# kalenforn/clip-based-cross-modal-hash

Measured on AMD Instinct MI355X. Metric: Hamming query x gallery pairs/sec (fused mAP@all pass, DCMHT COCO-shaped 64-bit), higher is better.
Workload: dtype u32; 1 GPU; configs[1] DCMHT COCO 64-bit retrieval: Q=5000 queries x R=117218 gallery items per GPU (x1 GPUs, contiguous shards), K=64 bits, C=80 classes, mAP@all; Q=5000, R_per_gpu=117218, K=64, C=80, parallelism=gallery-shard x1, query_blocks=1

## Files before the change

### clip-based-cross-modal-hash_amd/csrc/xmh_scan.hip

```cpp
#include "xmh_common.h"
#include <atomic>
#include <math.h>
#include <mutex>
#include <string.h>
#include <vector>
#include "xmh_scan_bits.h"
#include "xmh_scan_mfma.h"
#include "xmh_scan_kernels.h"

#include <stdlib.h>
#include <type_traits>

namespace {

constexpr int kSlotBudget64 = 9 * 1024;
constexpr int kSlotBudget32 = 5 * 1024;
constexpr int slots_for(int W, bool tern, int counter_bytes) {
    const int nbmax = (tern ? 64 : 32) * W + 1;
    const int budget = counter_bytes == 8 ? kSlotBudget64 : kSlotBudget32;
    const int cap = W > 8 ? 64 : 8;
    int S = 2;
    while (S < cap && nbmax * (64 / S) * counter_bytes > budget) S *= 2;
    return S;
}
// ... 350 lines not shown
        break;
    }
    case Kern::kApC: snprintf(out, n, "k_scan_ap_c<false, %d, %s>", l.eb, tf[l.half]); break;
    case Kern::kApR2: snprintf(out, n, "k_scan_ap_r2<%d, %d, %d, false>", l.nml, l.NW, l.S); break;
    }
    return XMH_OK;
}

int check_common(const char* who, const ScanCall& c, const xmh_scan_plan& p) {
    if (!c.qbits || !c.rbits || !c.qlab || !c.rlab || !c.ws) return xmh::fail(XMH_EINVAL, "%s: null pointer", who);
    if ((c.qzero == nullptr) != (c.rzero == nullptr)) return xmh::fail(XMH_EINVAL, "%s: zero masks must be given for both sides or neither", who);
    if (c.C <= 0) return xmh::fail(XMH_EINVAL, "%s: C=%d", who, c.C);
    const size_t need = ws_layout(p, 0).total;
    if (c.ws_bytes < need) return xmh::fail(XMH_EINVAL, "%s: workspace too small (%zu < %zu; %zu with the pair cache)", who, c.ws_bytes, need, (size_t)p.ws_bytes);
    return XMH_OK;
}

ScanArgs make_args(const ScanCall& c, const xmh_scan_plan& p) {
    return ScanArgs{c.qbits, c.qzero, c.qlab, c.rbits, c.rzero, c.rlab, (int)c.Q, (int)c.R, c.K, (int)p.chunk, (int)p.nchunk, (int)p.nqtile, (int)p.qpad,
                    (int)p.nbuckets, nullptr, (int)p.nqtile};
}

MfmaArgs r2_args(const ScanCall& c, const Launch& l, const xmh_scan_plan& p, int nqt) {
    MfmaArgs a{c.qbits, (int)c.Q, (int)c.R, c.K, l.W, (int)p.chunk, (int)p.nchunk, nqt, (int)p.nbuckets, (int)p.qpad};
    a.rbits = c.rbits; a.rlab = c.rlab; a.qlab = c.qlab; a.LW = l.LW;
    return a;
}

struct Geom { unsigned grid, block; size_t lds; int nqt, nrun; };
Geom launch_geom(const Launch& l, const xmh_scan_plan& p, int64_t Q) {
    const size_t nb = (size_t)p.nbuckets;
    const bool ap = l.kern == Kern::kApS || l.kern == Kern::kApC || l.kern == Kern::kApR2;
    Geom g{0, 64u * (unsigned)l.NW, 0, 0};
    if (l.kern == Kern::kHistS || l.kern == Kern::kApS) {
        g.lds = ((nb * (64 / l.S) * (ap && !l.p32 ? 2 : 1) + 3) & ~(size_t)3) * 4 * l.NW + (ap && l.cache ? 0 : aos_ring_bytes(l.W, l.LW, l.tern));
        g.nqt = (int)p.nqtile * l.S / l.NW;
    } else if (l.kern == Kern::kApC) {
        g.lds = nb * (64 / l.S) * 8; g.nqt = (int)p.nqtile * l.S;
    } else if (l.kern == Kern::kHistB) {
        g.nqt = (int)(p.qpad / (16 * kMfmaWaves));
    } else {
        g.lds = (size_t)l.NW * l.S * nb * 16 * (ap ? 8 : 4); g.nqt = (int)(p.qpad / (l.NW * l.S * 16));
    }
    g.nrun = g.nqt;
    if (ap) {
        static const bool all_tiles = xmh_experiment_env("XMH_AP_TILES") && atoi(xmh_experiment_env("XMH_AP_TILES")) == 0;
        if (!all_tiles) g.nrun = (int)xmh::ceil_div(Q, p.qpad / g.nqt);
    }
    g.grid = xmh::scan_grid_blocks(g.nrun, (int)p.nchunk);
    return g;
}

template <typename KernT, typename... Args>
int start(const char* who, const Launch& l, const Geom& g, hipStream_t st, KernT kern, int S, int NW, bool cache, Args... args) {
    if (l.S != S || l.NW != NW || l.cache != cache)
        return xmh::fail(XMH_ENOTSUP, "%s: the route names an instance with S=%d NW=%d cache=%d, the one compiled for W=%d LW=%d has S=%d NW=%d cache=%d", who, l.S,
                         l.NW, (int)l.cache, l.W, l.LW, S, NW, (int)cache);
    if (const int rc = xmh::raise_dynamic_lds(reinterpret_cast<const void*>(kern), g.lds, who)) return rc;
    hipLaunchKernelGGL(kern, dim3(g.grid), dim3(g.block), g.lds, st, args...);
    return XMH_OK;
}

struct ScanCtx {
    const ScanCall& c;
    hipStream_t st;
    xmh_scan_plan p;
    ScanRoute r;
    WsLayout L;
    ScanArgs a;
    uint32_t kcap = 0xffffffffu;
    bool capped = false;
    template <typename T> T* at(size_t off) const { return reinterpret_cast<T*>(static_cast<char*>(c.ws) + off); }
    uint32_t* chunk_hist() const { return at<uint32_t>(L.chunk_hist); }
    const uint2* below() const { return at<uint2>(L.below); }
    uint2* tot() const { return at<uint2>(L.tot); }
    uint2* dpre() const { return at<uint2>(L.dpre); }
    uint32_t* cap_ws() const { return at<uint32_t>(L.cap); }
    float* ap_part() const { return at<float>(L.ap_part); }
    ScanArgs args(const Geom& g, bool cached) const { ScanArgs as = a; as.nqt = g.nqt; as.nrun = g.nrun; as.pair_cache = cached ? pair_cache() : nullptr; return as; }
    uint32_t* gate(int word = 0) const { return at<uint32_t>(L.gate) + word; }
    const uint32_t* gate_if(const Launch& l, unsigned g, int word) const { return (l.gate & g) ? gate(word) : nullptr; }
    uint4* pair_cache() const { return r.cache_bytes ? at<uint4>(L.pair_cache) : nullptr; }
};

int plan_call(const char* who, ScanCtx& x, const Overrides& ov) {
    if (const int rc = make_plan(x.c.Q, x.c.R, x.c.K, x.c.tern, &x.p, ov)) return rc;
    return check_common(who, x.c, x.p);
}
void route_call(ScanCtx& x, Mode mode, const Overrides& ov) {
    x.r = scan_route(x.p, x.c, mode, ov, x.st);
    x.a = make_args(x.c, x.p);
    x.L = ws_layout(x.p, x.r.cache_bytes);
}

int valu_hist(const ScanCtx& x) {
    const Launch& h = x.r.p1;
    const Geom g = launch_geom(h, x.p, x.c.Q);
    const ScanArgs as = x.args(g, h.cache);
    auto go = [&](auto kern, int S, int NW, bool cache) {
        xmh::ProfScope prof("scan_hist", x.st);
        return start("xmh_hamming_hist", h, g, x.st, kern, S, NW, cache, as, x.chunk_hist());
    };
    auto launch = [&](auto tern_c) {
        constexpr bool T = decltype(tern_c)::value;
        return dispatch_shape<T>(h.W, h.LW, [&](auto w, auto l) {
            constexpr int WW = decltype(w)::value, LL = decltype(l)::value;
            if constexpr (kPairCacheShape<WW, T>) {
                if (h.cache) return go(k_scan_hist_s<WW, LL, T, cache_slots(WW), 1, true>, cache_slots(WW), 1, true);
            }
            constexpr int S = slots_for(WW, T, 4);
            constexpr int NW = S == 64 ? waves_for(WW, T) : 1;
            return go(k_scan_hist_s<WW, LL, T, S, NW, false>, S, NW, false);
        });
    };
    return h.tern ? launch(std::true_type{}) : launch(std::false_type{});
}

int mfma_hist(const ScanCtx& x) {
    const Launch& h = x.r.p1;
    const xmh_scan_plan& p = x.p;
    const Geom g = launch_geom(h, p, x.c.Q);
    uint32_t* chunk_hist = x.chunk_hist();
    uint4* cache = x.pair_cache();
    if (h.kern == Kern::kHistB) {
        xmh::ScanBitsArgs a{x.c.rbits, x.c.rlab, x.c.qbits, x.c.qlab, (int)x.c.Q, (int)x.c.R, x.c.K, h.W, h.LW, (int)p.chunk, (int)p.nchunk, g.nqt,
                            (int)p.nbuckets, (int)p.qpad};
        a.rzero = x.c.rzero; a.qzero = x.c.qzero;
        return xmh::launch_scan_hist_bits(a, h.S, chunk_hist, cache, x.st);
    }
    hipLaunchKernelGGL(k_scan_touch, dim3(xmh::scan_grid_blocks(kTouchPerChunk, (int)p.nchunk)), dim3(256), 0, x.st, x.c.rbits, x.c.rlab, x.c.R, h.W, h.LW,
                       p.chunk, (int)p.nchunk, x.at<uint32_t>(x.L.tick), (int)((x.L.gate + 256 - x.L.tick) / 4));
    XMH_LAUNCH_CHECK("xmh_hamming_hist control words");
    const MfmaArgs a = r2_args(x.c, h, p, g.nqt);
    xmh::ProfScope prof("scan_hist", x.st);
    auto go = [&](auto kern, int NW, int NQ, bool cached, auto... wrap_word) { return start("xmh_hamming_hist", h, g, x.st, kern, NQ, NW, cached, a, chunk_hist, cache, wrap_word...); };
    if (h.kern == Kern::kHistR2w) {
        uint32_t* ovf = x.gate(kGateWrapped);
        return h.nml == 1 ? (h.cache ? go(k_scan_hist_r2w<1, 4, 2, true>, 4, 2, true, ovf) : go(k_scan_hist_r2w<1, 4, 2, false>, 4, 2, false, ovf))
                          : (h.cache ? go(k_scan_hist_r2w<2, 4, 2, true>, 4, 2, true, ovf) : go(k_scan_hist_r2w<2, 4, 2, false>, 4, 2, false, ovf));
    }
    return h.nml == 1 ? (h.cache ? go(k_scan_hist_r2<1, 4, 4, true>, 4, 4, true) : go(k_scan_hist_r2<1, 4, 4, false>, 4, 4, false))
                      : (h.cache ? go(k_scan_hist_r2<2, 4, 4, true>, 4, 4, true) : go(k_scan_hist_r2<2, 4, 4, false>, 4, 4, false));
}

int hamming_hist_impl(const ScanCall& c, uint32_t* hist_all, uint32_t* hist_rel, xmh_stream_t stream, const Overrides& ov) {
    ScanCtx x{c, xmh::as_stream(stream)};
    if (const int rc = plan_call("xmh_hamming_hist", x, ov)) return rc;
    route_call(x, Mode::kUnsharded, ov);
    const xmh_scan_plan& p = x.p;
    const Kern kern = x.r.p1.kern;
    if (kern == Kern::kHistS || kern == Kern::kHistB) XMH_HIP(hipMemsetAsync(x.at<char>(x.L.tick), 0, x.L.gate + 256 - x.L.tick, x.st));
    if (const int rc = kern == Kern::kHistS ? valu_hist(x) : mfma_hist(x)) return rc;
    XMH_LAUNCH_CHECK("xmh_hamming_hist");
    hipLaunchKernelGGL(k_scan_below, dim3((unsigned)p.nqtile, (unsigned)xmh::ceil_div(p.nbuckets, 4)), dim3(256), 0, x.st, x.chunk_hist(), (int)p.qpad,
                       (int)p.nbuckets, (int)p.nchunk, kern != Kern::kHistS ? kRelHi16 : 0u, x.at<uint2>(x.L.below), x.tot(), x.at<uint32_t>(x.L.tick), (int)c.Q, x.dpre(),
                       x.cap_ws(), x.gate(), hist_all, hist_rel);
    XMH_LAUNCH_CHECK("xmh_hamming_hist below");
    return XMH_OK;
}

}

extern "C" int xmh_scan_plan_make(int64_t Q, int64_t R, int K, int ternary, xmh_scan_plan* plan_host) {
    if (!plan_host) return xmh::fail(XMH_EINVAL, "xmh_scan_plan_make: null plan");
    return make_plan(Q, R, K, ternary, plan_host);
}

extern "C" size_t xmh_scan_pair_cache_bytes(int64_t Q, int64_t R, int K, int ternary) {
    xmh_scan_plan p;
    if (make_plan(Q, R, K, ternary, &p)) return 0;
    return pair_cache_bytes(p, K, ternary != 0, pass1_family(K, ternary != 0, {}));
}

extern "C" size_t xmh_scan_pair_cache_offset(int64_t Q, int64_t R, int K, int ternary) {
    xmh_scan_plan p;
    if (make_plan(Q, R, K, ternary, &p)) return (size_t)-1;
    return ws_layout(p, 0).pair_cache;
}

extern "C" size_t xmh_scan_ws_bytes_nocache(int64_t Q, int64_t R, int K, int ternary) {
    xmh_scan_plan p;
    if (make_plan(Q, R, K, ternary, &p)) return 0;
    return ws_layout(p, 0).total;
}

extern "C" int xmh_scan_describe(int64_t Q, int64_t R, int K, int C, int ternary, char* out, size_t out_bytes) {
    if (!out || out_bytes < 64) return xmh::fail(XMH_EINVAL, "xmh_scan_describe: buffer too small");
    xmh_scan_plan p;
    if (const int rc = make_plan(Q, R, K, ternary, &p)) return rc;
    Overrides ov;
    ov.describe = true;
    const ScanCall c{nullptr, nullptr, nullptr, nullptr, nullptr, nullptr, Q, R, K, C, nullptr, (size_t)p.ws_bytes, ternary != 0};
    const ScanRoute r = scan_route(p, c, Mode::kUnsharded, ov, nullptr);
    char p1[160], p2[200] = "", one[120];
    if (const int rc = describe_launch(r.p1, p1, sizeof(p1))) return rc;
    for (const bool p32 : {true, false})
        for (int i = 0; i < r.n2; ++i) {
            if (r.p2[i].stand_in || r.p2[i].p32 != p32) continue;
            if (const int rc = describe_launch(r.p2[i], one, sizeof(one))) return rc;
            const size_t at = strlen(p2);
            snprintf(p2 + at, sizeof(p2) - at, "%s%s", at ? "|" : "", one);
        }
    if ((size_t)snprintf(out, out_bytes, "pass1=%s;pass2=%s", p1, p2) >= out_bytes) return xmh::fail(XMH_EINVAL, "xmh_scan_describe: buffer too small");
    return XMH_OK;
}

extern "C" int xmh_hamming_hist(const uint32_t* qbits, const uint32_t* qzero, const uint32_t* qlab,
                                const uint32_t* rbits, const uint32_t* rzero, const uint32_t* rlab, int64_t Q, int64_t R,
                                int K, int C, void* ws, size_t ws_bytes, uint32_t* hist_all, uint32_t* hist_rel,
                                xmh_stream_t stream) {
    XMH_RANGE("xmh_hamming_hist (pass 1)");
    const ScanCall c{qbits, qzero, qlab, rbits, rzero, rlab, Q, R, K, C, ws, ws_bytes, qzero != nullptr};
    return hamming_hist_impl(c, hist_all, hist_rel, stream, {});
}

namespace {
int ap_offsets(const ScanCtx& x, const Pass2& o) {
    const xmh_scan_plan& p = x.p;
    if (o.mode == Mode::kUnsharded) return XMH_OK;
    if (o.mode == Mode::kAllToAll)
        hipLaunchKernelGGL(k_shard_scatter_offsets, dim3((unsigned)xmh::ceil_div(p.qpad, 256), (unsigned)p.nbuckets + 1), dim3(256), 0, x.st,
                           reinterpret_cast<const uint2*>(o.hist_g), (int)p.nbuckets, (int)(p.qpad / o.world), (int)x.c.Q, (int)p.qpad, o.k, x.dpre(), x.cap_ws(),
                           o.cap, x.gate(2));
    else if (o.mode == Mode::kTotals)
        hipLaunchKernelGGL(k_shard_offsets_dpre, dim3((unsigned)p.nqtile), dim3(256), 0, x.st, reinterpret_cast<const uint2*>(o.hist_g), o.world, o.rank,
                           (int)x.c.Q, (int)p.qpad, (int)p.nbuckets, o.k, x.dpre(), x.cap_ws(), o.cap, x.gate(2));
    else
        hipLaunchKernelGGL(k_scan_dpre, dim3((unsigned)p.nqtile), dim3(256), 0, x.st, (const uint2*)x.tot(), (int)x.c.Q, (int)p.qpad, (int)p.nbuckets, o.base_all,
                           o.base_rel, o.nrel_total, o.k, x.dpre(), x.cap_ws(), o.cap, (uint32_t*)nullptr, (uint32_t*)nullptr, (uint32_t*)nullptr, x.gate(2));
    XMH_LAUNCH_CHECK(o.mode == Mode::kAllToAll ? "xmh_hamming_map_sharded_offsets scatter" : (o.mode == Mode::kTotals ? "xmh_hamming_map_sharded offsets" : "xmh_hamming_ap dpre"));
    return XMH_OK;
}

int ap_launch_c(const ScanCtx& x, const Launch& l) {
    const Geom g = launch_geom(l, x.p, x.c.Q);
    const ScanArgs as = x.args(g, true);
    xmh::ProfScope prof("scan_ap", x.st);
    auto go = [&](auto kc, int S) {
        return start("xmh_hamming_ap", l, g, x.st, kc, S, 1, l.cache, as, x.below(), (const uint2*)x.dpre(), (const uint32_t*)x.cap_ws(), x.ap_part(),
                     x.gate_if(l, kBySize, 2), x.kcap, x.gate_if(l, kByWrap, kGateWrapped), x.gate_if(l, kByWidth, 0), l.gate & kByWidth ? x.r.rank_bits : 0);
    };
    if (l.eb == 16) return x.capped ? go(k_scan_ap_c<true, 16>, 8) : go(k_scan_ap_c<false, 16>, 8);
    if (l.half) return x.capped ? go(k_scan_ap_c<true, 8, true>, 8) : go(k_scan_ap_c<false, 8, true>, 8);
    return x.capped ? go(k_scan_ap_c<true, 8>, 4) : go(k_scan_ap_c<false, 8>, 4);
}

int ap_launch_r2(const ScanCtx& x, const Launch& l) {
    const Geom g = launch_geom(l, x.p, x.c.Q);
    const MfmaArgs ma = r2_args(x.c, l, x.p, g.nrun);
    xmh::ProfScope prof("scan_ap", x.st);
    auto go = [&](auto kern) {
        return start("xmh_hamming_ap", l, g, x.st, kern, kAp2Groups, kAp2Waves, l.cache, ma, x.below(), (const uint2*)x.dpre(), (const uint32_t*)x.cap_ws(), x.ap_part(),
                     x.gate_if(l, kBySize, 2), x.kcap);
    };
    return l.nml == 1 ? (x.capped ? go(k_scan_ap_r2<1, kAp2Waves, kAp2Groups, true>) : go(k_scan_ap_r2<1, kAp2Waves, kAp2Groups, false>))
                      : (x.capped ? go(k_scan_ap_r2<2, kAp2Waves, kAp2Groups, true>) : go(k_scan_ap_r2<2, kAp2Waves, kAp2Groups, false>));
}

int ap_launch_s(const ScanCtx& x, const Launch& l) {
    const Geom g = launch_geom(l, x.p, x.c.Q);
    const ScanArgs as = x.args(g, l.cache);
    auto go = [&](auto kern, int S, int NW, bool cache, const uint32_t* run_if) {
        xmh::ProfScope prof(l.p32 ? "scan_ap32" : "scan_ap", x.st);
        return start("xmh_hamming_ap", l, g, x.st, kern, S, NW, cache, as, x.below(), (const uint2*)x.dpre(), (const uint32_t*)x.cap_ws(), x.ap_part(),
                     (const uint32_t*)x.gate(), x.r.rank_bits, x.kcap, x.gate_if(l, kBySize, 2), run_if);
    };
    auto by_shape = [&](auto tern_c, auto cap_c, auto p32_c, auto masked_c) {
        constexpr bool T = decltype(tern_c)::value, CP = decltype(cap_c)::value, P32 = decltype(p32_c)::value, MK = decltype(masked_c)::value;
        return dispatch_shape<T>(l.W, l.LW, [&](auto w, auto lw) {
            constexpr int WW = decltype(w)::value, LL = decltype(lw)::value;
            if constexpr (P32 && MK) return xmh::fail(XMH_ENOTSUP, "xmh_hamming_ap: the masked fallback runs 64-bit counters only");
            else {
                if constexpr (kPairCacheShape<WW, T> && !MK) {
                    if (l.cache)
                        return go(k_scan_ap_s<WW, 1, T, CP, cache_slots(WW), P32, MK, 1, true>, cache_slots(WW), 1, true, nullptr);
                }
                (void)CP;
                constexpr int S = slots_for(WW, T, P32 ? 4 : 8);
                constexpr int NW = S == 64 ? waves_for(WW, T) : 1;
                return go(k_scan_ap_s<WW, LL, T, true, S, P32, MK, NW, false>, S, NW, false, x.gate_if(l, kByWrap, kGateWrapped));
            }
        });
    };
    using T1 = std::true_type; using T0 = std::false_type;
    auto by_mask = [&](auto t, auto c, auto w) { return l.masked ? by_shape(t, c, w, T1{}) : by_shape(t, c, w, T0{}); };
    auto by_width = [&](auto t, auto c) { return l.p32 ? by_mask(t, c, T1{}) : by_mask(t, c, T0{}); };
    auto by_cap = [&](auto t) { return x.capped ? by_width(t, T1{}) : by_width(t, T0{}); };
    return l.tern ? by_cap(T1{}) : by_cap(T0{});
}

int ap_reduce(const ScanCtx& x, const Pass2& o) {
    const int64_t Q = x.c.Q;
    const unsigned nred = (unsigned)xmh::ceil_div(Q, 64);
    if (o.map_out && nred <= 4096) {
        hipLaunchKernelGGL(k_ap_reduce_map, dim3(nred), dim3(256), 0, x.st, (const float*)x.ap_part(), (int)Q, (int)x.p.qpad, (int)x.p.nchunk,
                           (const uint32_t*)x.cap_ws(), x.kcap, o.cap, o.ap_sum, x.at<double>(x.L.gate + 256), x.gate(1), o.map_out);
        XMH_LAUNCH_CHECK("xmh_hamming_map reduce+finalize");
        return XMH_OK;
    }
    hipLaunchKernelGGL(k_ap_reduce, dim3(nred), dim3(256), 0, x.st, (const float*)x.ap_part(), (int)Q, (int)x.p.qpad, (int)x.p.nchunk, o.ap_sum,
                       o.mode != Mode::kUnsharded ? (const uint32_t*)nullptr : (const uint32_t*)x.cap_ws(), x.kcap, o.cap);
    XMH_LAUNCH_CHECK("xmh_hamming_ap reduce");
    if (o.map_out) {
        hipLaunchKernelGGL(k_map_finalize, dim3(1), dim3(256), 0, x.st, (const double*)o.ap_sum, (const int32_t*)o.cap, Q, o.map_out);
        XMH_LAUNCH_CHECK("xmh_hamming_map finalize");
    }
    return XMH_OK;
// ... 243 lines not shown
```

### clip-based-cross-modal-hash_amd/csrc/xmh_scan_kernels.h

```cpp
#pragma once
#include "xmh_scan_mfma.h"

namespace {
template <int W, int LW, bool TERN>
struct QueryRegs {
    uint32_t b[W];
    uint32_t z[TERN ? W : 1];
    uint32_t l[LW];
    __device__ __forceinline__ void load(const ScanArgs& a, int q) {
        const bool ok = q < a.Q;
#pragma unroll
        for (int w = 0; w < W; ++w) b[w] = ok ? a.qbits[(int64_t)q * W + w] : 0u;
        if (TERN) {
#pragma unroll
            for (int w = 0; w < W; ++w) z[w] = ok ? a.qzero[(int64_t)q * W + w] : 0xffffffffu;
        }
#pragma unroll
        for (int w = 0; w < LW; ++w) l[w] = ok ? a.qlab[(int64_t)q * LW + w] : 0u;
    }
};

template <int W, int LW, bool TERN>
struct Rec {
    uint32_t b[W];
    uint32_t z[TERN ? W : 1];
    uint32_t l[LW];
};

template <int W, int LW, bool TERN>
__device__ __forceinline__ void rec_eval01(const QueryRegs<W, LW, TERN>& qr, const Rec<W, LW, TERN>& r, int K, int& d, uint32_t& hit01) {
    if (!TERN) {
        int acc = 0;
#pragma unroll
        for (int w = 0; w < W; ++w) acc += __popc(qr.b[w] ^ r.b[w]);
        d = acc;
    } else {
        int live_n = 0, diff_n = 0;
#pragma unroll
        for (int w = 0; w < W; ++w) {
            const uint32_t live = ~(qr.z[w] | r.z[w]);
            live_n += __popc(live);
            diff_n += __popc((qr.b[w] ^ r.b[w]) & live);
        }
        d = K - live_n + 2 * diff_n;
    }
    uint32_t hit = qr.l[0] & r.l[0];
#pragma unroll
    for (int w = 1; w < LW; ++w) asm("v_and_or_b32 %0, %1, %2, %0" : "+v"(hit) : "v"(qr.l[w]), "v"(r.l[w]));
    asm("v_min_u32 %0, %1, 1" : "=v"(hit01) : "v"(hit));
}

constexpr uint32_t kRelHi16 = 0xffffffffu;
constexpr int kGateWrapped = 3;
__global__ __launch_bounds__(256) void k_scan_below(const uint32_t* __restrict__ chunk_hist, int qpad, int nb, int nchunk, uint32_t rel_scale,
                                                    uint2* __restrict__ below, uint2* __restrict__ tot, uint32_t* __restrict__ tickets, int Q,
                                                    uint2* __restrict__ dpre, uint32_t* __restrict__ nrel_ws, uint32_t* __restrict__ nrel_max,
                                                    uint32_t* __restrict__ hist_all, uint32_t* __restrict__ hist_rel) {
    __shared__ uint2 part[4][64];
    __shared__ int last;
    const int lane = threadIdx.x & 63, wq = threadIdx.x >> 6;
    const int d = blockIdx.y * 4 + wq;
    const int q = blockIdx.x * 64 + lane;
    const bool hi16 = rel_scale == kRelHi16;
    if (d < nb) {
        uint32_t ra = 0, rr = 0;
        int c = 0;
        for (; c + 4 <= nchunk; c += 4) {
            uint32_t h[4];
#pragma unroll
            for (int j = 0; j < 4; ++j) h[j] = chunk_hist[((int64_t)(c + j) * nb + d) * qpad + q];
#pragma unroll
            for (int j = 0; j < 4; ++j) {
                below[((int64_t)(c + j) * nb + d) * qpad + q] = make_uint2(ra, rr);
                const uint32_t rel = hi16 ? h[j] & 0xffffu : (rel_scale ? h[j] / rel_scale : h[j] >> 16);
                ra += hi16 ? h[j] >> 16 : (rel_scale ? h[j] - rel * rel_scale : h[j] & 0xffffu);
                rr += rel;
            }
        }
        for (; c < nchunk; ++c) {
            const uint32_t h = chunk_hist[((int64_t)c * nb + d) * qpad + q];
            below[((int64_t)c * nb + d) * qpad + q] = make_uint2(ra, rr);
            const uint32_t rel = hi16 ? h & 0xffffu : (rel_scale ? h / rel_scale : h >> 16);
            ra += hi16 ? h >> 16 : (rel_scale ? h - rel * rel_scale : h & 0xffffu);
            rr += rel;
        }
        __hip_atomic_store(reinterpret_cast<unsigned long long*>(tot + (int64_t)d * qpad + q), (unsigned long long)ra | ((unsigned long long)rr << 32),
                           __ATOMIC_RELAXED, __HIP_MEMORY_SCOPE_AGENT);
    }
    if (!tickets) return;
    asm volatile("s_waitcnt vmcnt(0)" ::: "memory");
    __syncthreads();
    if (threadIdx.x == 0) {
        const uint32_t t = __hip_atomic_fetch_add(tickets + blockIdx.x, 1u, __ATOMIC_RELAXED, __HIP_MEMORY_SCOPE_AGENT);
        last = t == gridDim.y - 1;
    }
    __syncthreads();
    if (!last) return;
    auto tot_at = [&](int dd) {
        const unsigned long long v = __hip_atomic_load(reinterpret_cast<const unsigned long long*>(tot + (int64_t)dd * qpad + q), __ATOMIC_RELAXED,
                                                       __HIP_MEMORY_SCOPE_AGENT);
        return make_uint2((uint32_t)v, (uint32_t)(v >> 32));
    };
    const int nbq = (nb + 3) / 4;
    const int d0 = wq * nbq, d1 = (d0 + nbq < nb) ? d0 + nbq : nb;
    uint32_t sa = 0, sr = 0;
    for (int dd = d0; dd < d1; dd += 8) {
        uint2 t[8];
#pragma unroll
        for (int j = 0; j < 8; ++j) t[j] = dd + j < d1 ? tot_at(dd + j) : make_uint2(0u, 0u);
#pragma unroll
        for (int j = 0; j < 8; ++j) { sa += t[j].x; sr += t[j].y; }
    }
    part[wq][lane] = make_uint2(sa, sr);
    __syncthreads();
    uint32_t ra = 0, rr = 0, tr = 0;
#pragma unroll
    for (int w = 0; w < 4; ++w) {
        const uint2 pw = part[w][lane];
        if (w < wq) { ra += pw.x; rr += pw.y; }
        tr += pw.y;
    }
    for (int dd = d0; dd < d1; dd += 8) {
        uint2 t[8];
#pragma unroll
        for (int j = 0; j < 8; ++j) t[j] = dd + j < d1 ? tot_at(dd + j) : make_uint2(0u, 0u);
#pragma unroll
        for (int j = 0; j < 8; ++j) {
            if (dd + j < d1) {
                dpre[(int64_t)(dd + j) * qpad + q] = make_uint2(ra, rr);
                if (hist_all && q < Q) hist_all[(int64_t)q * nb + dd + j] = t[j].x;
                if (hist_rel && q < Q) hist_rel[(int64_t)q * nb + dd + j] = t[j].y;
                ra += t[j].x;
                rr += t[j].y;
            }
        }
    }
    if (wq == 0) {
        nrel_ws[q] = tr;
        if (q < Q) atomicMax(nrel_max, tr);
    }
}

__global__ __launch_bounds__(256) void k_scan_dpre(const uint2* __restrict__ tot, int Q, int qpad, int nb,
                                                   const uint32_t* __restrict__ base_all,
                                                   const uint32_t* __restrict__ base_rel,
                                                   const uint32_t* __restrict__ nrel_total, int64_t kcap,
                                                   uint2* __restrict__ dpre, uint32_t* __restrict__ cap_ws,
                                                   int32_t* __restrict__ cap_out, uint32_t* __restrict__ hist_all,
                                                   uint32_t* __restrict__ hist_rel, uint32_t* __restrict__ nrel_max,
                                                   uint32_t* __restrict__ rank_max = nullptr) {
    __shared__ uint2 part[4][64];
    const int lane = threadIdx.x & 63, wq = threadIdx.x >> 6;
    const int q = blockIdx.x * 64 + lane;
    const bool qok = q < Q;
    const int nbq = (nb + 3) / 4;
    const int d0 = wq * nbq, d1 = (d0 + nbq < nb) ? d0 + nbq : nb;
    uint32_t sa = 0, sr = 0;
    for (int d = d0; d < d1; d += 8) {
        uint2 t[8];
#pragma unroll
        for (int j = 0; j < 8; ++j) t[j] = d + j < d1 ? tot[(int64_t)(d + j) * qpad + q] : make_uint2(0u, 0u);
#pragma unroll
        for (int j = 0; j < 8; ++j) { sa += t[j].x; sr += t[j].y; }
    }
    part[wq][lane] = make_uint2(sa, sr);
    __syncthreads();
    uint32_t ra = 0, rr = 0, ta = 0, tr = 0, rmax = 0;
#pragma unroll
    for (int w = 0; w < 4; ++w) {
        const uint2 p = part[w][lane];
        if (w < wq) { ra += p.x; rr += p.y; }
        ta += p.x; tr += p.y;
    }
    for (int d = d0; d < d1; d += 8) {
        uint2 t[8];
#pragma unroll
        for (int j = 0; j < 8; ++j) t[j] = d + j < d1 ? tot[(int64_t)(d + j) * qpad + q] : make_uint2(0u, 0u);
#pragma unroll
        for (int j = 0; j < 8; ++j) {
            if (d + j < d1) {
                uint2 o = make_uint2(ra, rr);
                if (base_all && qok) {
                    o = make_uint2(base_all[(int64_t)q * nb + d + j], base_rel[(int64_t)q * nb + d + j]);
                    rmax = max(rmax, o.x + t[j].x);
                }
                if (dpre) dpre[(int64_t)(d + j) * qpad + q] = o;
                if (qok && hist_all) hist_all[(int64_t)q * nb + d + j] = t[j].x;
                if (qok && hist_rel) hist_rel[(int64_t)q * nb + d + j] = t[j].y;
                ra += t[j].x;
                rr += t[j].y;
            }
        }
    }
    if (cap_ws && wq == 0) {
        const uint32_t nrel = nrel_total ? (qok ? nrel_total[q] : 0u) : tr;
        const uint32_t cap = (kcap > 0 && (uint64_t)kcap < (uint64_t)nrel) ? (uint32_t)kcap : nrel;
        cap_ws[q] = nrel;
        if (qok && cap_out) cap_out[q] = (int32_t)cap;
        if (qok && nrel_max) atomicMax(nrel_max, nrel);
    }
    if (rank_max) {
        for (int o = 32; o; o >>= 1) rmax = max(rmax, (uint32_t)__shfl_xor((int)rmax, o));
        if (lane == 0 && rmax) atomicMax(rank_max, rmax);
    }
    (void)ta;
}

template <int W, int LW, bool TERN>
struct AosBatch {
    static constexpr int RW = W * (TERN ? 2 : 1) + LW;
    static constexpr int RS = (RW + 3) / 4 * 4;
    using R = Rec<W, LW, TERN>;
    static constexpr bool COAL = W >= 16 && !TERN;
    uint32_t w[RS];
    template <int NW = 1>
    __device__ __forceinline__ void load(const ScanArgs& a, int64_t base, int64_t hi, int lane, int wave = 0) {
        const int64_t i = base + lane;
        const bool ok = i < hi;
        if (COAL) {
#pragma unroll
            for (int jj = 0; jj < W / 4 / NW; ++jj) {
                const int o = (jj * NW + wave) * 256 + lane * 4;
                const bool okj = base + o / W < hi;
                const uint4 v = okj ? *reinterpret_cast<const uint4*>(a.rbits + base * W + o) : make_uint4(0u, 0u, 0u, 0u);
                w[4 * jj] = v.x; w[4 * jj + 1] = v.y; w[4 * jj + 2] = v.z; w[4 * jj + 3] = v.w;
            }
        } else {
#pragma unroll
            for (int x = 0; x < W; ++x) w[x] = ok ? a.rbits[i * W + x] : 0u;
        }
        if (TERN) {
#pragma unroll
            for (int x = 0; x < W; ++x) w[W + x] = ok ? a.rzero[i * W + x] : 0xffffffffu;
        }
        if (NW == 1 || wave == 0) {
#pragma unroll
            for (int x = 0; x < LW; ++x) w[W * (TERN ? 2 : 1) + x] = ok ? a.rlab[i * LW + x] : 0u;
        }
#pragma unroll
        for (int x = RW; x < RS; ++x) w[x] = 0u;
    }
    template <int NW = 1>
    __device__ __forceinline__ void publish(uint32_t* ring, int lane, int wave = 0) const {
        if (COAL) {
#pragma unroll
            for (int jj = 0; jj < W / 4 / NW; ++jj) {
                const int o = (jj * NW + wave) * 256 + lane * 4;
                *reinterpret_cast<uint4*>(ring + (o / W) * RS + (o % W)) = make_uint4(w[4 * jj], w[4 * jj + 1], w[4 * jj + 2], w[4 * jj + 3]);
            }
            if (NW == 1 || wave == 0)
                *reinterpret_cast<uint4*>(ring + lane * RS + W) = make_uint4(w[W], w[W + 1], w[W + 2], w[W + 3]);
            return;
        }
#pragma unroll
        for (int x = 0; x < RS; x += 4) *reinterpret_cast<uint4*>(ring + lane * RS + x) = make_uint4(w[x], w[x + 1], w[x + 2], w[x + 3]);
    }
    static __device__ __forceinline__ void get(R& r, const uint32_t* mine, int off_dwords) {
        uint32_t t[RS];
#pragma unroll
        for (int x = 0; x < RS; x += 4) {
            if (x + 4 <= RW || RW - x > 2) {
                const uint4 v = *reinterpret_cast<const uint4*>(mine + off_dwords + x);
                t[x] = v.x; t[x + 1] = v.y; t[x + 2] = v.z; t[x + 3] = v.w;
            } else if (RW - x == 2) {
                const uint2 v = *reinterpret_cast<const uint2*>(mine + off_dwords + x);
                t[x] = v.x; t[x + 1] = v.y; t[x + 2] = 0u; t[x + 3] = 0u;
            } else {
                t[x] = mine[off_dwords + x]; t[x + 1] = 0u; t[x + 2] = 0u; t[x + 3] = 0u;
            }
        }
#pragma unroll
        for (int x = 0; x < W; ++x) r.b[x] = t[x];
        if (TERN) {
#pragma unroll
            for (int x = 0; x < W; ++x) r.z[x] = t[W + x];
        }
#pragma unroll
        for (int x = 0; x < LW; ++x) r.l[x] = t[W * (TERN ? 2 : 1) + x];
    }
};

template <int S> struct SlotGeom {
    static constexpr int QW = 64 / S;
    static constexpr int LOG_QW = QW == 64 ? 6 : (QW == 32 ? 5 : (QW == 16 ? 4 : (QW == 8 ? 3 : (QW == 4 ? 2 : (QW == 2 ? 1 : 0)))));
    static constexpr int G = QW >= 16 ? 8 : (QW < 4 ? QW : 4);
    static constexpr int NG = QW / G;
};
// ... 670 lines not shown
```

Before: 1738 billion pairs/s.

## Widen k_scan_below to two queries per lane and batch chunk loads

Each lane in k_scan_below now handles two adjacent queries using uint2 loads and uint4 stores. Each wave covers two buckets, so the grid's y dimension halves. Chunk-histogram loads are issued in batches of 32 before a single vmcnt wait, and field extraction uses bitfield-extract instead of the divide/mask path. The last-block prefix pass loads all bucket totals once into registers when they fit, instead of reading tot twice. The intent is to raise memory-level parallelism and cut instruction and load overhead in this scan. In exchange it assumes the 16/16 packed format: the old general rel_scale divide path is replaced by shifts, and register pressure rises.

```diff
diff --git a/clip-based-cross-modal-hash_amd/csrc/xmh_scan.hip b/clip-based-cross-modal-hash_amd/csrc/xmh_scan.hip
--- a/clip-based-cross-modal-hash_amd/csrc/xmh_scan.hip
+++ b/clip-based-cross-modal-hash_amd/csrc/xmh_scan.hip
@@ -526,7 +526,7 @@
     if (kern == Kern::kHistS || kern == Kern::kHistB) XMH_HIP(hipMemsetAsync(x.at<char>(x.L.tick), 0, x.L.gate + 256 - x.L.tick, x.st));
     if (const int rc = kern == Kern::kHistS ? valu_hist(x) : mfma_hist(x)) return rc;
     XMH_LAUNCH_CHECK("xmh_hamming_hist");
-    hipLaunchKernelGGL(k_scan_below, dim3((unsigned)p.nqtile, (unsigned)xmh::ceil_div(p.nbuckets, 4)), dim3(256), 0, x.st, x.chunk_hist(), (int)p.qpad,
+    hipLaunchKernelGGL(k_scan_below, dim3((unsigned)p.nqtile, (unsigned)xmh::ceil_div(p.nbuckets, 8)), dim3(256), 0, x.st, x.chunk_hist(), (int)p.qpad,
                        (int)p.nbuckets, (int)p.nchunk, kern != Kern::kHistS ? kRelHi16 : 0u, x.at<uint2>(x.L.below), x.tot(), x.at<uint32_t>(x.L.tick), (int)c.Q, x.dpre(),
                        x.cap_ws(), x.gate(), hist_all, hist_rel);
     XMH_LAUNCH_CHECK("xmh_hamming_hist below");
diff --git a/clip-based-cross-modal-hash_amd/csrc/xmh_scan_kernels.h b/clip-based-cross-modal-hash_amd/csrc/xmh_scan_kernels.h
--- a/clip-based-cross-modal-hash_amd/csrc/xmh_scan_kernels.h
+++ b/clip-based-cross-modal-hash_amd/csrc/xmh_scan_kernels.h
@@ -51,6 +51,9 @@
 }
 
 constexpr uint32_t kRelHi16 = 0xffffffffu;
+constexpr int kBelowRound = 32;
+constexpr int kTotRound = 36;
+constexpr int kWaitVm0 = 0x0F70;
 constexpr int kGateWrapped = 3;
 __global__ __launch_bounds__(256) void k_scan_below(const uint32_t* __restrict__ chunk_hist, int qpad, int nb, int nchunk, uint32_t rel_scale,
                                                     uint2* __restrict__ below, uint2* __restrict__ tot, uint32_t* __restrict__ tickets, int Q,
@@ -58,34 +61,51 @@
                                                     uint32_t* __restrict__ hist_all, uint32_t* __restrict__ hist_rel) {
     __shared__ uint2 part[4][64];
     __shared__ int last;
-    const int lane = threadIdx.x & 63, wq = threadIdx.x >> 6;
-    const int d = blockIdx.y * 4 + wq;
-    const int q = blockIdx.x * 64 + lane;
-    const bool hi16 = rel_scale == kRelHi16;
-    if (d < nb) {
-        uint32_t ra = 0, rr = 0;
-        int c = 0;
-        for (; c + 4 <= nchunk; c += 4) {
-            uint32_t h[4];
-#pragma unroll
-            for (int j = 0; j < 4; ++j) h[j] = chunk_hist[((int64_t)(c + j) * nb + d) * qpad + q];
-#pragma unroll
-            for (int j = 0; j < 4; ++j) {
-                below[((int64_t)(c + j) * nb + d) * qpad + q] = make_uint2(ra, rr);
-                const uint32_t rel = hi16 ? h[j] & 0xffffu : (rel_scale ? h[j] / rel_scale : h[j] >> 16);
-                ra += hi16 ? h[j] >> 16 : (rel_scale ? h[j] - rel * rel_scale : h[j] & 0xffffu);
-                rr += rel;
-            }
-        }
-        for (; c < nchunk; ++c) {
-            const uint32_t h = chunk_hist[((int64_t)c * nb + d) * qpad + q];
-            below[((int64_t)c * nb + d) * qpad + q] = make_uint2(ra, rr);
-            const uint32_t rel = hi16 ? h & 0xffffu : (rel_scale ? h / rel_scale : h >> 16);
-            ra += hi16 ? h >> 16 : (rel_scale ? h - rel * rel_scale : h & 0xffffu);
-            rr += rel;
-        }
-        __hip_atomic_store(reinterpret_cast<unsigned long long*>(tot + (int64_t)d * qpad + q), (unsigned long long)ra | ((unsigned long long)rr << 32),
-                           __ATOMIC_RELAXED, __HIP_MEMORY_SCOPE_AGENT);
+    const int lane = threadIdx.x & 63, wq = __builtin_amdgcn_readfirstlane(threadIdx.x >> 6);
+    const uint32_t sh_all = rel_scale == kRelHi16 ? 16u : 0u, sh_rel = 16u - sh_all;
+    {
+        const int d = blockIdx.y * 8 + wq * 2 + (lane >> 5);
+        const int q2 = blockIdx.x * 64 + (lane & 31) * 2;
+        if (d < nb) {
+            const int64_t cs = (int64_t)nb * qpad;
+            const int64_t corner = (int64_t)blockIdx.y * 8 * qpad + blockIdx.x * 64;
+            const uint32_t off = (uint32_t)((wq * 2 + (lane >> 5)) * qpad + (lane & 31) * 2) * 4u;
+            const char* __restrict__ src = reinterpret_cast<const char*>(chunk_hist + corner);
+            char* __restrict__ dst = reinterpret_cast<char*>(below + corner);
+            int64_t step = cs * 4;
+            uint32_t a0 = 0, r0 = 0, a1 = 0, r1 = 0;
+            auto round = [&](int left) {
+                uint2 h[kBelowRound];
+#pragma unroll
+                for (int g = 0; g < kBelowRound; g += 8) {
+                    if (g < left) {
+#pragma unroll
+                        for (int j = g; j < g + 8; ++j) h[j] = *reinterpret_cast<const uint2*>(src + (j < left ? j : left - 1) * step + off);
+                    }
+                }
+                __builtin_amdgcn_s_waitcnt(kWaitVm0);
+#pragma unroll
+                for (int j = 0; j < kBelowRound; ++j) {
+                    if (j < left) {
+                        *reinterpret_cast<uint4*>(dst + 2 * j * step + 2u * off) = make_uint4(a0, r0, a1, r1);
+                        a0 += __builtin_amdgcn_ubfe(h[j].x, sh_all, 16);
+                        r0 += __builtin_amdgcn_ubfe(h[j].x, sh_rel, 16);
+                        a1 += __builtin_amdgcn_ubfe(h[j].y, sh_all, 16);
+                        r1 += __builtin_amdgcn_ubfe(h[j].y, sh_rel, 16);
+                    }
+                }
+                src += kBelowRound * step;
+                dst += 2 * kBelowRound * step;
+            };
+            round(nchunk);
+            for (int c0 = kBelowRound; c0 < nchunk; c0 += kBelowRound) {
+                asm volatile("" : "+s"(step));
+                round(nchunk - c0);
+            }
+            unsigned long long* t2 = reinterpret_cast<unsigned long long*>(tot + (int64_t)d * qpad + q2);
+            __hip_atomic_store(t2, (unsigned long long)a0 | ((unsigned long long)r0 << 32), __ATOMIC_RELAXED, __HIP_MEMORY_SCOPE_AGENT);
+            __hip_atomic_store(t2 + 1, (unsigned long long)a1 | ((unsigned long long)r1 << 32), __ATOMIC_RELAXED, __HIP_MEMORY_SCOPE_AGENT);
+        }
     }
     if (!tickets) return;
     asm volatile("s_waitcnt vmcnt(0)" ::: "memory");
@@ -96,43 +116,81 @@
     }
     __syncthreads();
     if (!last) return;
+    const int q = blockIdx.x * 64 + lane;
+    const uint32_t qoff = (uint32_t)lane * 8u;
+    const int64_t rowb = (int64_t)qpad * 8;
     auto tot_at = [&](int dd) {
-        const unsigned long long v = __hip_atomic_load(reinterpret_cast<const unsigned long long*>(tot + (int64_t)dd * qpad + q), __ATOMIC_RELAXED,
-                                                       __HIP_MEMORY_SCOPE_AGENT);
+        const char* row = reinterpret_cast<const char*>(tot + blockIdx.x * 64) + dd * rowb;
+        const unsigned long long v = __hip_atomic_load(reinterpret_cast<const unsigned long long*>(row + qoff), __ATOMIC_RELAXED, __HIP_MEMORY_SCOPE_AGENT);
         return make_uint2((uint32_t)v, (uint32_t)(v >> 32));
     };
     const int nbq = (nb + 3) / 4;
     const int d0 = wq * nbq, d1 = (d0 + nbq < nb) ? d0 + nbq : nb;
-    uint32_t sa = 0, sr = 0;
-    for (int dd = d0; dd < d1; dd += 8) {
-        uint2 t[8];
-#pragma unroll
-        for (int j = 0; j < 8; ++j) t[j] = dd + j < d1 ? tot_at(dd + j) : make_uint2(0u, 0u);
-#pragma unroll
-        for (int j = 0; j < 8; ++j) { sa += t[j].x; sr += t[j].y; }
-    }
-    part[wq][lane] = make_uint2(sa, sr);
-    __syncthreads();
-    uint32_t ra = 0, rr = 0, tr = 0;
-#pragma unroll
-    for (int w = 0; w < 4; ++w) {
-        const uint2 pw = part[w][lane];
-        if (w < wq) { ra += pw.x; rr += pw.y; }
-        tr += pw.y;
-    }
-    for (int dd = d0; dd < d1; dd += 8) {
-        uint2 t[8];
-#pragma unroll
-        for (int j = 0; j < 8; ++j) t[j] = dd + j < d1 ? tot_at(dd + j) : make_uint2(0u, 0u);
-#pragma unroll
-        for (int j = 0; j < 8; ++j) {
-            if (dd + j < d1) {
-                dpre[(int64_t)(dd + j) * qpad + q] = make_uint2(ra, rr);
-                if (hist_all && q < Q) hist_all[(int64_t)q * nb + dd + j] = t[j].x;
-                if (hist_rel && q < Q) hist_rel[(int64_t)q * nb + dd + j] = t[j].y;
-                ra += t[j].x;
-                rr += t[j].y;
-            }
+    uint32_t sa = 0, sr = 0, ra = 0, rr = 0, tr = 0;
+    auto exchange = [&]() {
+        part[wq][lane] = make_uint2(sa, sr);
+        __syncthreads();
+#pragma unroll
+        for (int w = 0; w < 4; ++w) {
+            const uint2 pw = part[w][lane];
+            if (w < wq) { ra += pw.x; rr += pw.y; }
+            tr += pw.y;
+        }
+    };
+    auto emit = [&](int dd, uint2 t, bool exports) {
+        *reinterpret_cast<uint2*>(reinterpret_cast<char*>(dpre + blockIdx.x * 64) + dd * rowb + qoff) = make_uint2(ra, rr);
+        if (exports && hist_all && q < Q) hist_all[(int64_t)q * nb + dd] = t.x;
+        if (exports && hist_rel && q < Q) hist_rel[(int64_t)q * nb + dd] = t.y;
+        ra += t.x;
+        rr += t.y;
+    };
+    const bool exports = hist_all || hist_rel;
+    if (nbq <= kTotRound) {
+        const int rows = d1 - d0;
+        uint2 t[kTotRound];
+#pragma unroll
+        for (int g = 0; g < kTotRound; g += 6) {
+            if (g < rows) {
+#pragma unroll
+                for (int j = g; j < g + 6; ++j) t[j] = tot_at(d0 + (j < rows ? j : rows - 1));
+            } else {
+#pragma unroll
+                for (int j = g; j < g + 6; ++j) t[j] = make_uint2(0u, 0u);
+            }
+        }
+        __builtin_amdgcn_s_waitcnt(kWaitVm0);
+#pragma unroll
+        for (int j = 0; j < kTotRound; ++j) {
+            if (j >= rows) t[j] = make_uint2(0u, 0u);
+            sa += t[j].x;
+            sr += t[j].y;
+        }
+        exchange();
+        if (exports) {
+#pragma unroll
+            for (int j = 0; j < kTotRound; ++j)
+                if (j < rows) emit(d0 + j, t[j], true);
+        } else {
+#pragma unroll
+            for (int j = 0; j < kTotRound; ++j)
+                if (j < rows) emit(d0 + j, t[j], false);
+        }
+    } else {
+        for (int dd = d0; dd < d1; dd += 8) {
+            uint2 t[8];
+#pragma unroll
+            for (int j = 0; j < 8; ++j) t[j] = dd + j < d1 ? tot_at(dd + j) : make_uint2(0u, 0u);
+#pragma unroll
+            for (int j = 0; j < 8; ++j) { sa += t[j].x; sr += t[j].y; }
+        }
+        exchange();
+        for (int dd = d0; dd < d1; dd += 8) {
+            uint2 t[8];
+#pragma unroll
+            for (int j = 0; j < 8; ++j) t[j] = dd + j < d1 ? tot_at(dd + j) : make_uint2(0u, 0u);
+#pragma unroll
+            for (int j = 0; j < 8; ++j)
+                if (dd + j < d1) emit(dd + j, t[j], true);
         }
     }
     if (wq == 0) {
```

After: 1752 billion pairs/s, median of 6. About the same (+0.8%).
